# inverted-ai/torchdriveenv

Measured on AMD Instinct MI355X. Metric: env-steps/sec, higher is better.
Workload: dtype f32

## Files before the change

### torchdriveenv_amd/csrc/tde_device.h

```cpp
#pragma once
#include <hip/hip_runtime.h>
#include <stdint.h>

#include "../../include/tde_abi.h"

#define TDE_DEV __device__ __forceinline__

typedef uint32_t u32x4_t __attribute__((ext_vector_type(4)));

namespace tde {

constexpr float kPi = 3.14159265358979323846f;
constexpr float kTwoPi = 6.28318530717958647692f;
constexpr float k2OverPi = 0.636619772367581343f;
constexpr float kPio2A = 1.5703125f;
constexpr float kPio2B = 4.837512969970703125e-4f;
constexpr float kPio2C = 7.54978995489188216e-8f;

TDE_DEV uint32_t mask_lo(unsigned long long m) { return (uint32_t)m; }
TDE_DEV uint32_t mask_hi(unsigned long long m) { return (uint32_t)(m >> 32); }
TDE_DEV bool upper_half(int i)
{
    int up = i & 32;
    asm("" : "+v"(up));
// ... 143 lines not shown

TDE_DEV float seg_d2_inv(float px, float py, float ax, float ay, float bx, float by, float inv)
{
    float abx = bx - ax, aby = by - ay;
    float apx = px - ax, apy = py - ay;
    float t = (apx * abx + apy * aby) * inv;
    t = clampf(t, 0.0f, 1.0f);
    float qx = apx - t * abx, qy = apy - t * aby;
    return qx * qx + qy * qy;
}

TDE_DEV float point_tri_d2_words(float px, float py, const float4 &t0, const float4 &t1, const float4 &t2)
{
    const float ax = t0.x, ay = t0.y, bx = t0.z, by = t0.w, cx = t1.x, cy = t1.y;
    float e0 = (bx - ax) * (py - ay) - (by - ay) * (px - ax);
    float e1 = (cx - bx) * (py - by) - (cy - by) * (px - bx);
    float e2 = (ax - cx) * (py - cy) - (ay - cy) * (px - cx);
    if ((e0 >= 0.0f && e1 >= 0.0f && e2 >= 0.0f) || (e0 <= 0.0f && e1 <= 0.0f && e2 <= 0.0f)) return 0.0f;
    float d = seg_d2_inv(px, py, ax, ay, bx, by, t1.z);
    d = fminf(d, seg_d2_inv(px, py, bx, by, cx, cy, t1.w));
    d = fminf(d, seg_d2_inv(px, py, cx, cy, ax, ay, t2.x));
    return d;
}

TDE_DEV float point_tri_d2_packed(float px, float py, const float4 *__restrict__ T)
{
    const float4 t0 = T[0], t1 = T[1];
    const float ax = t0.x, ay = t0.y, bx = t0.z, by = t0.w, cx = t1.x, cy = t1.y;
    float e0 = (bx - ax) * (py - ay) - (by - ay) * (px - ax);
    float e1 = (cx - bx) * (py - by) - (cy - by) * (px - bx);
    float e2 = (ax - cx) * (py - cy) - (ay - cy) * (px - cx);
    if ((e0 >= 0.0f && e1 >= 0.0f && e2 >= 0.0f) || (e0 <= 0.0f && e1 <= 0.0f && e2 <= 0.0f)) return 0.0f;
    const float inv_ca = T[2].x;
    float d = seg_d2_inv(px, py, ax, ay, bx, by, t1.z);
    d = fminf(d, seg_d2_inv(px, py, bx, by, cx, cy, t1.w));
    d = fminf(d, seg_d2_inv(px, py, cx, cy, ax, ay, inv_ca));
    return d;
}

TDE_DEV uint32_t cell_lookup(const tde_world &w, const tde_map &m, float px, float py)
{
    const float fx = __builtin_amdgcn_fmed3f((px - m.ox) * m.inv_cell, 0.0f, (float)(m.nx - 1));
    const float fy = __builtin_amdgcn_fmed3f((py - m.oy) * m.inv_cell, 0.0f, (float)(m.ny - 1));
    return w.cell_word[(uint32_t)m.cell_base + (((uint32_t)(int)fy << m.row_shift) + (uint32_t)(int)fx)];
}

template <typename T> TDE_DEV T sel4(int i, T a0, T a1, T a2, T a3)
{
    const bool b0 = (i & 1) != 0, b1 = (i & 2) != 0;
    const T lo = b0 ? a1 : a0, hi = b0 ? a3 : a2;
    return b1 ? hi : lo;
}
#define TDE_SEL4(i, a0, a1, a2, a3) sel4((i), (a0), (a1), (a2), (a3))

struct Corners {
    float px0, py0, px1, py1, px2, py2, px3, py3;
    uint32_t w0, w1, w2, w3;
};

TDE_DEV uint32_t cell_class_lookup(const tde_world &w, const tde_map &m, float px, float py)
{
    const float fx = __builtin_amdgcn_fmed3f((px - m.ox) * m.inv_cell, 0.0f, (float)(m.nx - 1));
    const float fy = __builtin_amdgcn_fmed3f((py - m.oy) * m.inv_cell, 0.0f, (float)(m.ny - 1));
    const uint32_t ix = (uint32_t)(int)fx, iy = (uint32_t)(int)fy;
    const uint32_t tile = (uint32_t)m.cls2_base + ((iy >> 4) << (m.row_shift - 5)) + (ix >> 5);
    const uint32_t word = w.cell_cls2[(tile << 5) | (((iy & 15u) << 1) | ((ix >> 4) & 1u))];
    return ((word >> ((ix & 15u) << 1)) & 3u) | (((uint32_t)m.cell_base + ((iy << m.row_shift) + ix)) << 2);
}

#ifndef TDE_STEP_CLS2
#define TDE_STEP_CLS2 1
#endif
#ifndef TDE_ROLLOUT_CLS2
#define TDE_ROLLOUT_CLS2 0
#endif

template <bool CLS2 = false>
TDE_DEV void offroad_issue(const tde_world &w, const tde_map &m, bool live, float x, float y, float c, float s, float hl,
                           float hw, Corners &k)
{
    const float lx = hl * c, ly = hl * s, wx = hw * s, wy = hw * c;
    k.px0 = (x + lx) - wx; k.py0 = (y + ly) + wy;
    k.px1 = (x + lx) + wx; k.py1 = (y + ly) - wy;
    k.px2 = (x - lx) + wx; k.py2 = (y - ly) - wy;
    k.px3 = (x - lx) - wx; k.py3 = (y - ly) + wy;
    k.w0 = k.w1 = k.w2 = k.w3 = TDE_CELL_FULL;
    if (live) {
        if constexpr (CLS2) {
            k.w0 = cell_class_lookup(w, m, k.px0, k.py0);
            k.w1 = cell_class_lookup(w, m, k.px1, k.py1);
            k.w2 = cell_class_lookup(w, m, k.px2, k.py2);
            k.w3 = cell_class_lookup(w, m, k.px3, k.py3);
        } else {
            k.w0 = cell_lookup(w, m, k.px0, k.py0);
            k.w1 = cell_lookup(w, m, k.px1, k.py1);
            k.w2 = cell_lookup(w, m, k.px2, k.py2);
            k.w3 = cell_lookup(w, m, k.px3, k.py3);
        }
    }
}

template <bool PAIR = false, bool CLS2 = false>
TDE_DEV bool offroad_resolve(const tde_world &w, const Corners &k, float thr2, int rec_base)
{
    const uint32_t w0 = k.w0, w1 = k.w1, w2 = k.w2, w3 = k.w3;
    static_assert(TDE_CELL_EMPTY == 0u && TDE_CELL_MIXED == 1u && TDE_CELL_FULL == 2u, "cell classes");
    bool off = min(min(w0 & 3u, w1 & 3u), min(w2 & 3u, w3 & 3u)) == 0u;
    uint32_t pending = off ? 0u : ((w0 & 1u) | ((w1 & 1u) << 1) | ((w2 & 1u) << 2) | ((w3 & 1u) << 3));
    bool work = false;
    uint32_t cur = 0, end = 0;
    float qx = 0.0f, qy = 0.0f;
    const float4 *recs = reinterpret_cast<const float4 *>(w.cell_tri);
    for (;;) {
        if (!work && pending) {
            const int ci = __ffs((int)pending) - 1;
            pending &= pending - 1u;
            uint32_t wd = TDE_SEL4(ci, w0, w1, w2, w3);
            if constexpr (CLS2) wd = w.cell_word[wd >> 2];
            cur = (wd >> 10) + (uint32_t)rec_base;
            end = cur + ((wd >> 2) & 255u);
            qx = TDE_SEL4(ci, k.px0, k.px1, k.px2, k.px3);
            qy = TDE_SEL4(ci, k.py0, k.py1, k.py2, k.py3);
            work = true;
        }
        if (!__ballot(work)) break;
        if (work) {
            if constexpr (PAIR) {
                const float4 *r0 = recs + 3 * (size_t)cur, *r1 = recs + 3 * (size_t)(cur + 1 < end ? cur + 1 : cur);
                const float4 a0 = r0[0], a1 = r0[1], a2 = r0[2], b0 = r1[0], b1 = r1[1], b2 = r1[2];
                bool on = point_tri_d2_words(qx, qy, a0, a1, a2) <= thr2;
                if (!on && cur + 1 < end) on = point_tri_d2_words(qx, qy, b0, b1, b2) <= thr2;
                cur += 2;
                if (on) work = false;
                else if (cur >= end) { off = true; work = false; pending = 0u; }
            } else {
                const float d2 = point_tri_d2_packed(qx, qy, recs + 3 * (size_t)cur);
                if (d2 <= thr2) work = false;
                else if (++cur == end) { off = true; work = false; pending = 0u; }
            }
        }
    }
    return off;
}

template <bool PAIR = false, bool CLS2 = false>
TDE_DEV bool box_offroad(const tde_world &w, const tde_map &m, bool live, float x, float y, float c, float s, float hl,
                         float hw, float thr2)
{
    Corners k;
    offroad_issue<CLS2>(w, m, live, x, y, c, s, hl, hw, k);
    return offroad_resolve<PAIR, CLS2>(w, k, thr2, m.rec_base);
}

TDE_DEV uint4 philox(uint64_t seed, uint32_t c0, uint32_t c1, uint32_t c2, uint32_t c3)
{
    uint32_t k0 = (uint32_t)seed, k1 = (uint32_t)(seed >> 32);
#pragma unroll
    for (int r = 0; r < 10; ++r) {
        uint32_t h0 = __umulhi(0xD2511F53u, c0), l0 = 0xD2511F53u * c0;
        uint32_t h1 = __umulhi(0xCD9E8D57u, c2), l1 = 0xCD9E8D57u * c2;
        uint32_t n0 = h1 ^ c1 ^ k0, n2 = h0 ^ c3 ^ k1;
        c0 = n0; c1 = l1; c2 = n2; c3 = l0;
        k0 += 0x9E3779B9u; k1 += 0xBB67AE85u;
    }
    return make_uint4(c0, c1, c2, c3);
}

TDE_DEV double u01(uint32_t r) { return (double)(r >> 8) * (1.0 / 16777216.0); }

struct Sliver { double lo, hi; };
__host__ TDE_DEV Sliver sliver_of(double r) { const double r2 = r * r; return Sliver{r2 * (1.0 - 1e-12), r2 * (1.0 + 1e-12)}; }
TDE_DEV bool sqrt_gt(double s, double r, const Sliver &v)
{
    if (s > v.hi) return true;
    if (s < v.lo) return false;
    return sqrt(s) > r;
}
TDE_DEV bool sqrt_ge(double s, double r, const Sliver &v)
{
    if (s > v.hi) return true;
    if (s < v.lo) return false;
    return sqrt(s) >= r;
}

TDE_DEV double cos_kernel_f64(double x, double y)
{
    const double z = x * x;
    const double r = z * __builtin_fma(z, __builtin_fma(z, __builtin_fma(z, __builtin_fma(z, __builtin_fma(z,
                         -1.13596475577881948265e-11, 2.08757232129817482790e-09), -2.75573143513906633035e-07),
                         2.48015872894767294178e-05), -1.38888888888741095749e-03), 4.16666666666666019037e-02);
    const double hz = 0.5 * z, w = 1.0 - hz;
    return w + (((1.0 - w) - hz) + (z * r - x * y));
}
TDE_DEV double sin_kernel_f64(double x, double y)
{
    const double z = x * x, v = z * x;
    const double r = __builtin_fma(z, __builtin_fma(z, __builtin_fma(z, __builtin_fma(z, 1.58969099521155010221e-10,
                         -2.50507602534068634195e-08), 2.75573137070700676789e-06), -1.98412698298579493134e-04),
                         8.33333333332248946124e-03);
    return x - ((z * (0.5 * y - v * r) - y) - v * -1.66666666666666324348e-01);
}
TDE_DEV double cos_heading_f64(double x)
{
    if (__builtin_fabs(x) < 0.78539816339744830962) return cos_kernel_f64(x, 0.0);
    const double fn = __builtin_rint(x * 6.36619772367581382433e-01);
    const int n = (int)fn;
    const double r = x - fn * 1.57079632673412561417e+00, w = fn * 6.07710050650619224932e-11;
    const double y0 = r - w, y1 = (r - y0) - w;
    const double v = (n & 1) ? sin_kernel_f64(y0, y1) : cos_kernel_f64(y0, y1);
    return (((n + 1) & 2) != 0) ? -v : v;
}

__host__ TDE_DEV void cut2f_bounds(double r, float &lo, float &hi)
{
    const double r2 = r * r;
    lo = 0.0f; hi = __builtin_inff();
    if (r2 > 1e-30 && r2 < 1e30) { lo = (float)(r2 * (1.0 - 1e-6)); hi = (float)(r2 * (1.0 + 1e-6)); }
}

struct Cold {
    double waypoint_bonus, heading_penalty, distance_bonus, distance_cutoff, reach_radius;
    Sliver cut_sliver, reach_sliver;
    float cut2f_lo, cut2f_hi;
    uint64_t seed;
    const tde_spawn *spawn;
    const tde_scenario *scn;
    const double *wp_xy;
    const tde_map *maps;
    const float *route_xy;
    const float *start_psi;
    uint32_t env_base;
    int n_scn, NW, RW, max_steps, terminated_at_infraction, NH;
};

__host__ TDE_DEV void fill_cold(Cold &c, const tde_config &cfg, const tde_world &w)
{
    c.waypoint_bonus = cfg.waypoint_bonus; c.heading_penalty = cfg.heading_penalty;
    c.distance_bonus = cfg.distance_bonus; c.distance_cutoff = cfg.distance_cutoff;
    c.reach_radius = cfg.reach_radius; c.seed = cfg.seed;
    c.cut_sliver = sliver_of(cfg.distance_cutoff); c.reach_sliver = sliver_of(cfg.reach_radius);
    cut2f_bounds(cfg.distance_cutoff, c.cut2f_lo, c.cut2f_hi);
    c.spawn = w.spawn; c.scn = w.scn; c.wp_xy = w.wp_xy; c.maps = w.maps; c.route_xy = w.route_xy;
    c.start_psi = w.start_psi; c.NH = w.NH;
    c.env_base = cfg.env_base; c.n_scn = w.n_scn; c.NW = w.NW; c.RW = w.RW;
    c.max_steps = cfg.max_steps; c.terminated_at_infraction = cfg.terminated_at_infraction;
}

struct RewardBounds { Sliver cut, reach; float cut2f_lo, cut2f_hi; };
TDE_DEV RewardBounds reward_bounds(const Cold &c) { return RewardBounds{c.cut_sliver, c.reach_sliver, c.cut2f_lo, c.cut2f_hi}; }
TDE_DEV RewardBounds reward_bounds(const tde_config &c)
{
    RewardBounds b{sliver_of(c.distance_cutoff), sliver_of(c.reach_radius), 0.0f, 0.0f};
    cut2f_bounds(c.distance_cutoff, b.cut2f_lo, b.cut2f_hi);
    return b;
}

struct RewardOut {
    float reward;
    uint8_t terminated, truncated;
    double psi_smooth, speed_smooth, psi_r, dist_r;
};

template <typename CFG>
TDE_DEV double reward_dist_term(const CFG &cfg, const RewardBounds &rb, float lx, float ly, float x, float y)
{
    const float fdx = x - lx, fdy = y - ly;
    const float s32 = fdx * fdx + fdy * fdy;
    bool moved = s32 > rb.cut2f_hi;
    if (!moved && !(s32 < rb.cut2f_lo)) {
        const double ddx = (double)x - (double)lx, ddy = (double)y - (double)ly;
        moved = sqrt_gt(ddx * ddx + ddy * ddy, cfg.distance_cutoff, rb.cut);
    }
    return moved ? cfg.distance_bonus : 0.0;
}
template <typename CFG> TDE_DEV double reward_psi_term(const CFG &cfg, float lpsi, float psi)
{
    const float dpsi = psi - lpsi;
    return (1.0 - cos_heading_f64((double)dpsi)) * (-cfg.heading_penalty);
}
template <typename CFG>
TDE_DEV void reward_motion_terms(const CFG &cfg, const RewardBounds &rb, float lx, float ly, float lpsi, float x, float y,
                                 float psi, double &dist_r, double &psi_r)
{
    dist_r = reward_dist_term(cfg, rb, lx, ly, x, y);
    psi_r = reward_psi_term(cfg, lpsi, psi);
}
template <typename CFG>
TDE_DEV bool reward_reach(const CFG &cfg, const RewardBounds &rb, float x, float y, double wtx, double wty)
{
    const double tx = (double)x - wtx, ty = (double)y - wty;
    return !sqrt_ge(tx * tx + ty * ty, cfg.reach_radius, rb.reach);
}
template <typename CFG> TDE_DEV float reward_sum(const CFG &cfg, bool reach, double dist_r, double psi_r)
{
    return (float)(((reach ? cfg.waypoint_bonus : 0.0) + dist_r) + psi_r);
}

template <typename CFG>
TDE_DEV RewardOut reward_core(const CFG &cfg, int n_wp, double wtx, double wty, float lx, float ly, float lpsi,
                              float lv, float x, float y, float psi, float v, bool off, bool col, bool tl, int k,
                              int &target_idx, int &reached, bool want_info = true)
{
    RewardOut o;
    const RewardBounds rb = reward_bounds(cfg);
    reward_motion_terms(cfg, rb, lx, ly, lpsi, x, y, psi, o.dist_r, o.psi_r);
    const int ti = target_idx;
// ... 16 lines not shown
```

### torchdriveenv_amd/csrc/tde_kernels.h

```cpp
#ifndef TDE_KERNELS_H
#define TDE_KERNELS_H
#include <hip/hip_runtime.h>
#include <stdint.h>
#include <stdio.h>
#include <stdlib.h>
#include <string.h>
#include <atomic>
#include <type_traits>

#include "../../include/tde_hip.h"
#include "tde_device.h"
#include "tde_magnitudes.h"
#include "tde_raster.h"

#if (defined(TDE_EXP_NO_COLL_MAG) || defined(TDE_EXP_NO_OFF_MAG) || defined(TDE_EXP_EXTRA_LOAD) || defined(TDE_EXP_NO_D_RESPAWN) || \
     defined(TDE_EXP_NO_C_RESPAWN) || (defined(TDE_EXP_MAG_FRAME) && TDE_EXP_MAG_FRAME != 0)) && !defined(TDE_EXPERIMENT_BUILD)
#error "TDE_EXP_* switches build a library that computes WRONG results (timing experiments): add -DTDE_EXPERIMENT_BUILD to say you mean it"
#endif

namespace tde {

constexpr int kBlock = 256;
constexpr int kWave = 64;

// ... 1738 lines not shown
                if (F & TDE_F_REWARD) {
                    const float4 pa = sh.a[q][0], pc = sh.c[q][0];
                    int n_target = er.target_idx, n_reached = er.reached;
                    rw = reward_core(cold, cx.n_wp, cx.wtx, cx.wty, pa.x, pa.y, pc.x, pc.y, x, y, rc.x, rc.y, false, false, false, k,
                                     n_target, n_reached, st.info != nullptr);
                    const bool advanced = n_target != er.target_idx;
                    er.target_idx = n_target; er.reached = n_reached;
                    if (st.info) {
                        double *inf = st.info + 4 * (int64_t)e;
                        inf[0] = rw.psi_smooth; inf[1] = rw.speed_smooth; inf[2] = rw.psi_r; inf[3] = rw.dist_r;
                    }
                    if (st.info_reached) st.info_reached[e] = er.reached;
                    if (advanced) load_ego_target(cold, er, cx);
                    o.terminated = (uint8_t)(cold.terminated_at_infraction && (off || hit || tl));
                    o.truncated = (uint8_t)(k >= cold.max_steps);
                    done = (o.terminated | o.truncated) ? 1 : 0;
                }
                sh.done = ((F & TDE_F_REWARD) && (F & TDE_F_AUTORESET)) ? done : 0;
                if (ro.reward) ro.reward[(int64_t)i * LB + e] = rw.reward;
                if (ro.done)
                    ro.done[(int64_t)i * LB + e] =
                        (uint8_t)(o.terminated | (o.truncated << 1) | (o.offroad << 2) | (o.collided << 3) | (o.tl << 4));
            }
        }
        lds_barrier();
        const bool respawned = sh.done != 0;
        if (respawned) reset_lane<A>(cfg, cold, e, a, ag, er);
        st.collided[g] = respawned ? 0 : o.collided;
        st.offroad[g] = respawned ? 0 : o.offroad;
        if (a == 0) {
            st.scn[e] = er.scn; st.episode[e] = er.episode;
            st.steps[e] = er.steps;
            st.target_idx[e] = er.target_idx;
            st.reached[e] = er.reached;
            st.reward[e] = rw.reward;
            st.terminated[e] = o.terminated;
            st.truncated[e] = o.truncated;
            if (st.tl_violation) st.tl_violation[e] = o.tl;
        }
    } else if (NW == 8 && role == 2) {
        __builtin_amdgcn_s_setprio(3);
        if (lane == 0) sh.help_seq[wv & 1] = 0;
        lds_barrier();
        for (int i = 0; i < ro.K; ++i) {
            const int q = (i & 1) ^ 1;
            if (F & TDE_F_NPC) {
                const float4 ra = sh.a[q][a], rb = sh.b[q][a];
                const float gf = sh.ctl[a];
                Agent me{};
                me.x = ra.x; me.y = ra.y; me.len = 2.0f * rb.z;
                const unsigned long long own = one_bit64(63 - (a & 63));
                sh.gap_part[a] = npc_gap<64>(cfg, &sh.a[q][64], &sh.b[q][64], a - 64, a < 64 ? 0ull : own, me, rb.x, rb.y, gf >= 0.0f, gf);
                asm volatile("s_waitcnt lgkmcnt(0)" ::: "memory");
                if (lane == 0) *reinterpret_cast<volatile int *>(&sh.help_seq[wv & 1]) = i + 1;
            }
            lds_barrier();
            if (sh.done && first_acts) lds_barrier();
            lds_barrier();
        }
        lds_barrier();
    } else if (NW == 8 && role == 3) {
        __builtin_amdgcn_s_setprio(1);
        Agent ag{};
        EnvRegs er{st.scn[e], st.steps[e], st.target_idx[e], st.reached[e], st.episode[e]};
        RedCache redc; redc.invalidate();
        tde_map m{};
        if (F & (TDE_F_OFFROAD | TDE_F_TRAFFIC_LIGHTS)) m = cold.maps[reinterpret_cast<const int4 *>(cold.scn)[er.scn].x];
        const float thr2 = thr2_of(cfg);
        if (lane == 0) sh.off_seq[wv & 1] = 0;
        lds_barrier();
        for (int i = 0; i < ro.K; ++i) {
            const int p = i & 1;
            lds_barrier();
            if (sh.done) {
                reset_lane<A>(cfg, cold, e, a, ag, er);
                if (F & (TDE_F_OFFROAD | TDE_F_TRAFFIC_LIGHTS)) m = cold.maps[reinterpret_cast<const int4 *>(cold.scn)[er.scn].x];
                redc.invalidate();
                if (first_acts) lds_barrier();
            }
            lds_barrier();
            er.steps += 1;
            const float4 ra = sh.a[p][a], rb = sh.b[p][a], rc = sh.c[p][a];
            const bool live = rc.z != 0.0f;
            bool off = false;
            if (F & TDE_F_OFFROAD) {
                Corners corners;
                offroad_issue<false>(w, m, live, ra.x, ra.y, rb.x, rb.y, rb.z, rb.w, corners);
                off = offroad_resolve<false, false>(w, corners, thr2, m.rec_base);
            }
            sh.offw[a] = off ? 1 : 0;
            if (LIGHTS && (F & TDE_F_TRAFFIC_LIGHTS) && a == 0)
                sh.tlw = tl_violation_of(WideLines{sh, w.stoplines + m.stop_base}, m.n_stop, red_mask_cached(w, m, er.steps, redc), ra.x, ra.y, rb.x, rb.y, rb.z, rb.w) ? 1 : 0;
            asm volatile("s_waitcnt lgkmcnt(0)" ::: "memory");
            if (lane == 0) *reinterpret_cast<volatile int *>(&sh.off_seq[wv & 1]) = i + 1;
        }
        lds_barrier();
    }
}
#undef TDE_WIDE_PROLOGUE

#ifdef TDE_DEBUG
#ifndef TDE_DUMMY_D
#define TDE_DUMMY_D 0
#endif
#ifndef TDE_DUMMY_C
#define TDE_DUMMY_C 0
#endif
#ifndef TDE_DUMMY_O
#define TDE_DUMMY_O 0
#endif
#ifndef TDE_DUMMY_ILP
#define TDE_DUMMY_ILP 1
#endif
template <int N> TDE_DEV void dummy_valu(float seed)
{
    if constexpr (N > 0) {
        float v[TDE_DUMMY_ILP];
#pragma unroll
        for (int u = 0; u < TDE_DUMMY_ILP; ++u) v[u] = seed + (float)u;
#pragma unroll
        for (int n = 0; n < N / TDE_DUMMY_ILP; ++n) {
#pragma unroll
            for (int u = 0; u < TDE_DUMMY_ILP; ++u) asm volatile("v_fma_f32 %0, %0, %0, %0" : "+v"(v[u]));
        }
#pragma unroll
        for (int u = 0; u < TDE_DUMMY_ILP; ++u) asm volatile("" :: "v"(v[u]));
    }
}
#define TDE_PROBE(N, seed) dummy_valu<N>(seed)
#else
#define TDE_PROBE(N, seed) ((void)0)
#endif
#ifndef TDE_STEP_PRIO_SWITCH
#define TDE_STEP_PRIO_SWITCH 1
#endif
#ifndef TDE_STEP_PRIO_D2
#define TDE_STEP_PRIO_D2 0
#define TDE_STEP_PRIO_C2 3
#define TDE_STEP_PRIO_O2 2
#endif
#ifndef TDE_SPRIO_C
#define TDE_SPRIO_C 0
#define TDE_SPRIO_O 1
#endif
#ifndef TDE_PRIO_D
#define TDE_PRIO_D 2
#define TDE_PRIO_C 0
#define TDE_PRIO_O 1
#endif
#ifndef TDE_ROLLOUT_CONST_ARGS
#define TDE_ROLLOUT_CONST_ARGS 0
#endif
struct RolloutArgs { tde_config cfg; tde_world w; tde_state st; tde_rollout ro; uint32_t act_hash; };
#if TDE_ROLLOUT_CONST_ARGS
__constant__ RolloutArgs g_rollout_args;
#endif
template <int A, bool LIGHTS, bool BIG>
__global__ __launch_bounds__(3 * kWave) __attribute__((amdgpu_waves_per_eu(6, 6))) void env_rollout_trio_kernel(
#if TDE_ROLLOUT_CONST_ARGS
    int unused_)
{
    const tde_config &cfg = g_rollout_args.cfg; const tde_world &w = g_rollout_args.w; const tde_state &st = g_rollout_args.st;
    const tde_rollout &ro = g_rollout_args.ro;
    const uint32_t act_hash = g_rollout_args.act_hash;
#else
    tde_config cfg, tde_world w, tde_state st, tde_rollout ro, uint32_t act_hash)
{
#endif
    __shared__ DuoShared sh;
    __shared__ Cold cold;
    const int lane = threadIdx.x & (kWave - 1);
    const int role = __builtin_amdgcn_readfirstlane((int)(threadIdx.x >> 6));
    if (threadIdx.x == 0) {
        fill_cold(cold, cfg, w); sh.done = 0ull; sh.hit_mask = 0ull; sh.off_mask = 0ull; sh.tl_mask = 0ull;
        sh.max_steps_w = cfg.max_steps; sh.term_at_infraction_w = cfg.terminated_at_infraction;
        sh.red_seq = -1;
    }
    const uint32_t F = cfg.flags;
    const bool lights = LIGHTS && (F & TDE_F_TRAFFIC_LIGHTS);
    constexpr bool kGapCache = TDE_FIRST_GAP != 0 && LIGHTS;
    const bool first_acts = (F & TDE_F_NPC_FIRST_STEP) != 0;
    const int64_t g = (int64_t)blockIdx.x * kWave + lane;
    const int e = (int)(g / A), a = (int)(g % A);
    const int B = st.B;
    const int LB = ro.ldb;
    const bool valid = e < B;
    const int64_t gs = valid ? g : 0;
    const int es = valid ? e : 0;
    const int base = lane - a;
    __syncthreads();
#define TDE_ROLE_PROLOGUE                                                                                 \
    Agent ag;                                                                                             \
    load_agent(st, gs, ag);                                                                               \
    if (!valid) ag.present = false;                                                                       \
    EnvRegs er{st.scn[es], st.steps[es], st.target_idx[es], st.reached[es], st.episode[es]};              \
    Ctx cx;                                                                                               \
    load_ctx<A>(cfg, cold, a, ag, er, cx);

    uint4 m0, m1;
    auto done_of = [&](int k, unsigned long long &term_m, unsigned long long &trunc_m) {
        const unsigned long long ego = __ballot(a == 0 && valid);
        m0 = *reinterpret_cast<const uint4 *>(&sh.hit_mask);
        m1 = *reinterpret_cast<const uint4 *>(&sh.tl_mask);
        const unsigned long long infr = (((unsigned long long)(m0.y | m0.w | m1.y)) << 32) | (m0.x | m0.z | m1.x);
        term_m = ((F & TDE_F_REWARD) && m1.w) ? (infr & ego) : 0ull;
        trunc_m = (F & TDE_F_REWARD) ? __ballot(a == 0 && valid && k >= (int)m1.z) : 0ull;
        return ((F & TDE_F_REWARD) && (F & TDE_F_AUTORESET)) ? (term_m | trunc_m) : 0ull;
    };
    if (role == 0) {
        TDE_ROLE_PROLOGUE
        __builtin_amdgcn_s_setprio(TDE_PRIO_D);
        float c0, s0;
        sincos_f32(ag.psi, s0, c0);
        write_rows(sh, 1, lane, valid && ag.present, ag, c0, s0, cfg.npc_lane_half);
        lds_barrier();
        for (int i = 0; i < ro.K; ++i) {
            const int p = i & 1, q = p ^ 1;
            const float2 act = sh.act[p][base];
            float nx, ny, npsi, nv, nc, ns;
            float na = 0.0f, nb = 0.0f;
            int nwp, k;
            bool switched, live;
            bool again = false;
            for (int pass = 0;; ++pass) {
                k = er.steps + 1;
                live = valid && ag.present;
                const bool npc = (F & TDE_F_NPC) && a > 0 && live;
                const bool replayed = (F & TDE_F_REPLAY) && a > 0 && live && k < cx.replay_len;
                float4 rep = make_float4(0.0f, 0.0f, 0.0f, 0.0f);
                if (replayed) rep = reinterpret_cast<const float4 *>(w.replay_states)[(int64_t)ag.replay * w.RT + k];
                const bool has_target = npc && ag.route >= 0 && ag.route_wp < cx.route_n;
                float acc = 0.0f, beta = 0.0f;
                if (a == 0) { acc = act.x; beta = act.y; }
                if (F & TDE_F_NPC) {
                    if (pass == 0 || again) {
                        const float gap = npc_gap<A>(cfg, &sh.a[q][base], &sh.b[q][base], a, bit_of_row<A>(a), ag, c0, s0, has_target, cx.g_far);
                        float red_gap = 1e30f;
                        if (lights) {
                            if (pass == 0) {
                                while (*reinterpret_cast<volatile int *>(&sh.red_seq) != i) __builtin_amdgcn_s_sleep(1);
                                red_gap = *reinterpret_cast<volatile float *>(&sh.red_gap[p][lane]);
                            } else if (has_target) {
                                const tde_map m = cold.maps[reinterpret_cast<const int4 *>(cold.scn)[er.scn].x];
                                const uint32_t red = red_mask(w, m, k);
                                if (red) red_gap = red_line_gap_of<GlobalLines, 1>(cfg, GlobalLines{w.stoplines + m.stop_base}, m.n_stop, red, ag, c0, s0);
                            }
                        }
                        npc_act_of_gap(cfg, ag, c0, s0, has_target, cx.tgx, cx.tgy, gap, has_target ? red_gap : 1e30f, na, nb);
                    }
                    if (npc && (k > 1 || first_acts)) { acc = na; beta = nb; }
                }
                nx = ag.x; ny = ag.y; npsi = ag.psi; nv = ag.v;
                if (live) {
                    bicycle(nx, ny, npsi, nv, ag.inv_lr, acc, beta, cfg.dt);
                    if (replayed) { nx = rep.x; ny = rep.y; npsi = rep.z; nv = rep.w; }
                }
                switched = false;
                nwp = ag.route_wp;
                if (has_target) {
                    const float dx = cx.tgx - nx, dy = cx.tgy - ny;
                    if (dx * dx + dy * dy < cfg.npc_reach * cfg.npc_reach) { nwp += 1; switched = true; }
                }
                sincos_f32(npsi, ns, nc);
                TDE_PROBE(TDE_DUMMY_D, nx);
                if (pass) break;
                lds_barrier();
                unsigned long long term_m, trunc_m;
                const unsigned long long dn = i > 0 ? done_of(er.steps, term_m, trunc_m) : 0ull;
                if (lane == 0) sh.done = dn;
                if (!dn) break;
                const bool fresh = mask_bit(dn, base) && valid;
                uint2 fg_ent = make_uint2(0u, 0u);
                if (fresh) {
                    reset_lane<A>(cfg, cold, e, a, ag, er);
                    if (kGapCache && first_acts && (F & TDE_F_NPC) && a > 0 && w.first_gap)
                        fg_ent = *reinterpret_cast<const uint2 *>(w.first_gap + ((int64_t)er.scn * A + a));
                    load_ctx<A>(cfg, cold, a, ag, er, cx);
                    sincos_f32(ag.psi, s0, c0);
                    write_rows(sh, q, lane, ag.present, ag, c0, s0, cfg.npc_lane_half);
                }
                if (first_acts && (F & TDE_F_NPC)) {
                    again = true;
                    if constexpr (kGapCache) {
                        const bool f_npc = fresh && a > 0 && ag.present;
                        const bool f_target = f_npc && ag.route >= 0 && ag.route_wp < cx.route_n;
                        again = !npc_first_step<A>(cfg, fg_ent, first_gap_key(act_hash), &sh.a[q][base], &sh.b[q][base], a, ag, c0, s0, f_npc, f_target,
                                                   cx.tgx, cx.tgy, na, nb);
                    }
                }
            }
            ag.x = nx; ag.y = ny; ag.psi = npsi; ag.v = nv; ag.route_wp = nwp;
            c0 = nc; s0 = ns;
            er.steps = k;
            write_rows(sh, p, lane, live, ag, c0, s0, cfg.npc_lane_half);
            lds_barrier();
            if (switched) load_route_target(cold, ag, cx);
        }
        lds_barrier();
        {
            unsigned long long term_m, trunc_m;
            const unsigned long long dn = done_of(er.steps, term_m, trunc_m);
            if (lane == 0) sh.done = dn;
            lds_barrier();
            if (mask_bit(dn, base) && valid) reset_lane<A>(cfg, cold, e, a, ag, er);
        }
        if (!valid) return;
        store_agent_dynamic(st, g, ag);
        store_agent_static(st, g, ag);
    } else if (role == 1) {
        __builtin_amdgcn_s_setprio(TDE_PRIO_C);
        TDE_ROLE_PROLOGUE
        RedCache redc; redc.invalidate();
        bool hit = false;
        uint8_t last_term = 0, last_trunc = 0;
        int npend = 0, ipend0 = 0;
        const bool batch = (F & TDE_F_REWARD) != 0;
        if (batch) load_ego_ctx(cold, er, cx);
        auto flush = [&](bool final) {
            const int n = npend;
            if (n == 0) return;
            const bool act = valid && a < n;
            const float4 r0 = sh.ring_pre[lane], r1 = sh.ring_post[lane];
            const RewardBounds rbn = reward_bounds(cold);
            double dist_r = 0.0, psi_r = 0.0;
            if (act) reward_motion_terms(cold, rbn, r0.x, r0.y, r0.z, r1.x, r1.y, r1.z, dist_r, psi_r);
            int from = 0;
            for (;;) {
                bool reach = false;
                if (act && a >= from && er.target_idx < cx.n_wp) reach = reward_reach(cold, rbn, r1.x, r1.y, cx.wtx, cx.wty);
                const unsigned long long rm = __ballot(reach);
                const uint32_t envbits = mask_field(rm, base) & (A >= 32 ? 0xffffffffu : ((1u << (A & 31)) - 1u));
                const int s1 = envbits ? __ffs((int)envbits) - 1 : A;
                if (act && a >= from && a <= s1) {
                    const float rwd = reward_sum(cold, a == s1, dist_r, psi_r);
                    if (ro.reward) ro.reward[(int64_t)(ipend0 + a) * LB + e] = rwd;
                    if (final && a == n - 1) {
                        st.reward[e] = rwd;
                        if (st.info) {
                            double *inf = st.info + 4 * (int64_t)e;
                            inf[0] = (double)fabsf((r0.z - r1.z) / 0.1f); inf[1] = (double)fabsf((r0.w - r1.w) / 0.1f);
                            inf[2] = psi_r; inf[3] = dist_r;
                        }
                    }
                }
                bool more = false;
                if (s1 < A) {
                    er.target_idx += 1; er.reached += 1;
                    load_ego_target(cold, er, cx);
                    from = s1 + 1;
                    more = valid && from < n;
                } else {
                    from = n;
                }
                if (!__ballot(more)) break;
            }
            if (final && a == 0 && valid && st.info_reached) st.info_reached[e] = er.reached;
            ipend0 += n; npend = 0;
        };
        auto settle = [&](int i) {
            unsigned long long term_m, trunc_m;
            const unsigned long long dn = done_of(er.steps, term_m, trunc_m);
            if (a == 0 && valid) {
                last_term = (uint8_t)mask_bit(term_m, lane); last_trunc = (uint8_t)mask_bit(trunc_m, lane);
                if (ro.done) {
                    const bool up = lane >= 32;
                    const uint32_t sft = (uint32_t)lane & 31u;
                    const uint32_t hb = ((up ? m0.y : m0.x) >> sft) & 1u, ob = ((up ? m0.w : m0.z) >> sft) & 1u,
                                   tb = ((up ? m1.y : m1.x) >> sft) & 1u;
                    ro.done[(int64_t)i * LB + e] = (uint8_t)(last_term | (last_trunc << 1) | (ob << 2) | (hb << 3) | (tb << 4));
                }
            }
            return dn;
        };
        auto publish_red_gaps = [&](int step, int buf, int kk) {
            __builtin_amdgcn_s_setprio(3);
            const float4 ra = sh.a[buf][lane], rb = sh.b[buf][lane];
            float rg = 1e30f;
            const uint32_t red = red_mask_cached(w, cx.m, kk, redc);
            if (red) {
                Agent me{};
                me.x = ra.x; me.y = ra.y; me.len = 2.0f * rb.z;
                if (cx.m.n_stop <= kStopCache)
                    rg = red_line_gap_of<CacheOnlyLines<A>, TDE_JUDGE_GAP_LINES>(cfg, CacheOnlyLines<A>{sh, lane / A}, cx.m.n_stop, red, me, rb.x, rb.y);
                else
                    rg = red_line_gap_of<CachedLines<A>, TDE_JUDGE_GAP_LINES>(cfg, CachedLines<A>{sh, w.stoplines + cx.m.stop_base, lane / A}, cx.m.n_stop, red, me, rb.x, rb.y);
            }
            sh.red_gap[step & 1][lane] = rg;
            if (a == 0) sh.lights2[step & 1][lane / A] = make_int4((int)red, 0, cx.m.stop_base, cx.m.n_stop);
            asm volatile("s_waitcnt lgkmcnt(0)" ::: "memory");
            if (lane == 0) *reinterpret_cast<volatile int *>(&sh.red_seq) = step;
            __builtin_amdgcn_s_setprio(TDE_PRIO_C);
        };
        if (lights) fill_stop_cache<A>(sh, w, cx.m, lane, a);
        lds_barrier();
        if (lights) publish_red_gaps(0, 1, er.steps + 1);
        for (int i = 0; i < ro.K; ++i) {
            const int p = i & 1, q = p ^ 1;
            lds_barrier();
            if (i > 0) {
                const unsigned long long dn = settle(i - 1);
                if (dn && batch) flush(false);
                if (dn && mask_bit(dn, base) && valid) {
                    reset_lane<A>(cfg, cold, e, a, ag, er);
                    load_ctx<A>(cfg, cold, a, ag, er, cx);
                    if (batch) load_ego_ctx(cold, er, cx);
                    redc.invalidate();
                    if (lights) {
                        fill_stop_cache<A>(sh, w, cx.m, lane, a);
                        if (a == 0) sh.lights2[p][lane / A] = make_int4((int)red_mask_cached(w, cx.m, 1, redc), 0, cx.m.stop_base, cx.m.n_stop);
                    }
                }
            }
            lds_barrier();
            er.steps += 1;
            const int k = er.steps;
            if (lights && i + 1 < ro.K) publish_red_gaps(i + 1, p, k + 1);
            const float4 ra = sh.a[p][lane], rb = sh.b[p][lane], rc = sh.c[p][lane];
            if constexpr (A == 16 && TDE_COLLIDE_DPP)
                hit = collide_rows_dpp16(&sh.a[p][base], &sh.b[p][base], a, rc.z != 0.0f, ra.x, ra.y, rb.x, rb.y, rb.z, rb.w, ra.z);
            else
                hit = collide_rows<A>(&sh.a[p][base], &sh.b[p][base], a, rc.z != 0.0f, ra.x, ra.y, rb.x, rb.y, rb.z, rb.w, ra.z);
            const unsigned long long m = __ballot(hit);
            if (lane == 0) sh.hit_mask = m;
            TDE_PROBE(TDE_DUMMY_C, ra.x);
            if (batch) {
                if (a == 0 && valid) {
                    const float4 pa = sh.a[q][lane], pc = sh.c[q][lane];
                    sh.ring_pre[lane + npend] = make_float4(pa.x, pa.y, pc.x, pc.y);
                    sh.ring_post[lane + npend] = make_float4(ra.x, ra.y, rc.x, rc.y);
                }
                npend += 1;
                if (npend == A && i + 1 < ro.K) flush(false);
            } else if (a == 0 && valid && ro.reward) {
                ro.reward[(int64_t)i * LB + e] = 0.0f;
            }
        }
        lds_barrier();
        settle(ro.K - 1);
        if (batch) flush(true);
        lds_barrier();
        const bool respawned = mask_bit(sh.done, base) != 0;
        if (respawned && valid) reset_lane<A>(cfg, cold, e, a, ag, er);
        if (!valid) return;
        st.collided[g] = respawned ? 0 : (hit ? 1 : 0);
        if (a == 0) {
            st.scn[e] = er.scn; st.episode[e] = er.episode;
            st.steps[e] = er.steps;
            st.target_idx[e] = er.target_idx;
            st.reached[e] = er.reached;
            if (!batch) st.reward[e] = 0.0f;
            st.terminated[e] = last_term;
            st.truncated[e] = last_trunc;
        }
    } else {
        __builtin_amdgcn_s_setprio(TDE_PRIO_O);
        TDE_ROLE_PROLOGUE
        const float thr2 = thr2_of(cfg);
        bool off = false, tl = false;
        const float2 *acts = reinterpret_cast<const float2 *>(ro.actions);
        const bool ego = a == 0 && valid;
        if (ego) {
            sh.act[0][lane] = acts[e];
            sh.act[1][lane] = acts[(int64_t)(ro.K > 1 ? 1 : 0) * LB + e];
        }
        lds_barrier();
        for (int i = 0; i < ro.K; ++i) {
            const int p = i & 1;
            float2 act2 = make_float2(0.0f, 0.0f);
            if (ego) act2 = acts[(int64_t)(i + 2 < ro.K ? i + 2 : ro.K - 1) * LB + e];
            lds_barrier();
            lds_barrier();
            if (i > 0) {
                const unsigned long long dn = sh.done;
                if (dn && mask_bit(dn, base) && valid) {
                    reset_lane<A>(cfg, cold, e, a, ag, er);
                    load_ctx<A>(cfg, cold, a, ag, er, cx);
                }
            }
            er.steps += 1;
            const int k = er.steps;
            const float4 ra = sh.a[p][lane], rb = sh.b[p][lane], rc = sh.c[p][lane];
            const bool live = rc.z != 0.0f;
            off = false;
            if (F & TDE_F_OFFROAD) off = box_offroad<false, BIG || TDE_ROLLOUT_CLS2>(w, cx.m, live, ra.x, ra.y, rb.x, rb.y, rb.z, rb.w, thr2);
            tl = false;
            if (lights && a == 0 && valid) {
                const int4 lw = sh.lights2[p][lane / A];
                if (lw.w <= kStopCache) tl = tl_violation_of(CacheOnlyLines<A>{sh, lane / A}, lw.w, (uint32_t)lw.x, ra.x, ra.y, rb.x, rb.y, rb.z, rb.w);
                else tl = tl_violation_of(CachedLines<A>{sh, w.stoplines + lw.z, lane / A}, lw.w, (uint32_t)lw.x, ra.x, ra.y, rb.x, rb.y, rb.z, rb.w);
            }
            TDE_PROBE(TDE_DUMMY_O, ra.x);
            const unsigned long long om = __ballot(off), tm = __ballot(tl);
            if (lane == 0) { sh.off_mask = om; sh.tl_mask = tm; }
            if (ego) sh.act[p][lane] = act2;
        }
        lds_barrier();
        lds_barrier();
        if (!valid) return;
        st.offroad[g] = mask_bit(sh.done, base) ? 0 : (off ? 1 : 0);
        if (a == 0 && st.tl_violation) st.tl_violation[e] = tl ? 1 : 0;
    }
}
#undef TDE_ROLE_PROLOGUE

TDE_DEV void load_next_target(const Cold &w, const Agent &ag, int route_n, float &x2, float &y2)
{
    x2 = y2 = 0.0f;
    if (ag.route >= 0 && ag.route_wp + 1 < route_n) {
        const float2 tg = reinterpret_cast<const float2 *>(w.route_xy)[(int64_t)ag.route * w.RW + ag.route_wp + 1];
        x2 = tg.x; y2 = tg.y;
    }
}

constexpr uint32_t kSlotKeyFlags = TDE_F_NPC | TDE_F_REPLAY;
constexpr int kSlotTg2Later = 1 << 29;

TDE_DEV int slot_key(const Agent &ag, uint32_t F)
{
    return (ag.route_wp & 0xFFFF) | (int)((F & kSlotKeyFlags) << 16) | TDE_CACHE_VALID;
}

template <int A>
TDE_DEV void load_ctx_cached(const tde_config &cfg, const Cold &cold, const tde_state &st, int64_t g, int a, bool valid,
                             const int4 &s0, const int4 &s1, Agent &ag, const EnvRegs &er, Ctx &cx,
                             bool want_map, bool &rebuilt)
{
    const uint32_t F = cfg.flags;
    const bool hit = !valid || (s0.x == er.scn && (s0.y & ~kSlotTg2Later) == slot_key(ag, F));
    rebuilt = !hit;
    cx.wtx = cx.wty = 0.0; cx.n_wp = 0;
    cx.tgx2 = cx.tgy2 = 0.0f;
    if (__ballot(!hit)) {
        if (!hit) {
            load_ctx<A>(cfg, cold, a, ag, er, cx);
            load_next_target(cold, ag, cx.route_n, cx.tgx2, cx.tgy2);
        }
    }
    if (hit) {
        cx.tgx = __int_as_float(s0.z); cx.tgy = __int_as_float(s0.w);
        constexpr uint32_t idm = (1u << TDE_CACHE_ID_BITS) - 1u;
        ag.route = (int)((uint32_t)s1.x & idm) - 1; cx.route_n = (int)((uint32_t)s1.x >> TDE_CACHE_ID_BITS);
        ag.replay = (int)((uint32_t)s1.y & idm) - 1; cx.replay_len = (int)((uint32_t)s1.y >> TDE_CACHE_ID_BITS);
        cx.tgx2 = __int_as_float(s1.z); cx.tgy2 = __int_as_float(s1.w);
        cx.g_far = (ag.vdes * ag.vdes / cfg.npc_max_accel) * 1.01f + cfg.npc_gap_s0 + 0.1f;
        if (want_map && (F & (TDE_F_OFFROAD | TDE_F_TRAFFIC_LIGHTS))) {
            const int4 e0 = reinterpret_cast<const int4 *>(st.env_cache + (g / A))[0];
            const int map = ((e0.z & TDE_CACHE_VALID) && e0.x == er.scn) ? e0.w : reinterpret_cast<const int4 *>(cold.scn)[er.scn].x;
            cx.m = cold.maps[map];
        }
    }
}

TDE_DEV void store_slot_cache(const tde_state &st, int64_t g, const Agent &ag, const EnvRegs &er, const Ctx &cx, uint32_t F,
                              bool tg2_later = false)
{
    static_assert(sizeof(tde_slot_cache) == 32, "two 16-byte words per slot");
    int4 *sc4 = reinterpret_cast<int4 *>(st.slot_cache + g);
    sc4[0] = make_int4(er.scn, slot_key(ag, F) | (tg2_later ? kSlotTg2Later : 0), __float_as_int(cx.tgx), __float_as_int(cx.tgy));
    sc4[1] = make_int4((int)((uint32_t)(ag.route + 1) | ((uint32_t)cx.route_n << TDE_CACHE_ID_BITS)),
                       (int)((uint32_t)(ag.replay + 1) | ((uint32_t)cx.replay_len << TDE_CACHE_ID_BITS)),
                       __float_as_int(cx.tgx2), __float_as_int(cx.tgy2));
}

TDE_DEV int act_key_steps(uint32_t cfg_hash, int steps) { return (int)(cfg_hash ^ ((uint32_t)steps * 0x9E3779B1u)); }


#ifndef TDE_WIDE_PRIO_D2
#define TDE_WIDE_PRIO_D2 3
#endif
#ifndef TDE_WIDE_PRIO_J2
#define TDE_WIDE_PRIO_J2 1
#endif
#ifndef TDE_WIDE4_SWEEP_BLOCK
#define TDE_WIDE4_SWEEP_BLOCK 4
#endif
#ifndef TDE_WIDE_STEP_WAVES8
#define TDE_WIDE_STEP_WAVES8 1
#endif
struct WideStepShared : WideShared {
    int early[2];
    float poly[32];
};

template <bool LIGHTS, bool OBS, bool MAG, int NW = 4>
__global__ __launch_bounds__(NW * kWave) __attribute__((amdgpu_waves_per_eu(4, 4))) void env_step_wide_kernel(const StepArgs *__restrict__ args,
                                                                                                           const float *__restrict__ action)
{
    const tde_config &cfg = args->cfg;
    const tde_world &w = args->w;
    const tde_state &st = args->st;
    const uint32_t act_hash = args->act_hash;
    constexpr int A = 128;
    __shared__ WideStepShared sh;
#if TDE_WIDE_COLD_IN_BLOCK
    const Cold &cold = args->cold;
#define TDE_WIDE_COLD_BARRIER() ((void)0)
#else
    __shared__ Cold cold;
#define TDE_WIDE_COLD_BARRIER() lds_barrier()
#endif
    const int lane = threadIdx.x & (kWave - 1);
    const int wv = wide_role_wave();
    const int role = wv >> 1;
    const int a = ((wv & 1) << 6) | lane;
#if !TDE_WIDE_COLD_IN_BLOCK
    if (wv == (NW == 8 ? 4 : 2) && lane == 0) fill_cold(cold, cfg, w);
#endif
    const uint32_t F = cfg.flags;
    const bool first_acts = (F & TDE_F_NPC_FIRST_STEP) != 0;
    const bool lights = LIGHTS && (F & TDE_F_TRAFFIC_LIGHTS);
    const int e = (int)blockIdx.x;
    const int64_t g = (int64_t)e * A + a;
    if (role == 0) {
        __builtin_amdgcn_s_setprio(2);
        Agent ag;
        load_agent(st, g, ag);
        EnvRegs er{st.scn[e], st.steps[e], st.target_idx[e], st.reached[e], st.episode[e]};
        const float2 act = reinterpret_cast<const float2 *>(action)[e];
        float2 ac = make_float2(0.0f, 0.0f);
        int2 akey = make_int2(-1, 0);
        float2 *ap = st.act_cache ? reinterpret_cast<float2 *>(st.act_cache) + (int64_t)e * (A + 1) : nullptr;
        if (ap) { ac = ap[a]; akey = reinterpret_cast<const int2 *>(ap)[A]; }
        int4 sc0 = make_int4(0, 0, 0, 0), sc1 = sc0;
        if (st.slot_cache) { sc0 = reinterpret_cast<const int4 *>(st.slot_cache + g)[0]; sc1 = reinterpret_cast<const int4 *>(st.slot_cache + g)[1]; }
        TDE_WIDE_COLD_BARRIER();
        Ctx cx;
        bool rebuilt;
        load_ctx_cached<A>(cfg, cold, st, g, a, true, sc0, sc1, ag, er, cx, false, rebuilt);
        if (!rebuilt && lights) cx.m = cold.maps[reinterpret_cast<const int4 *>(cold.scn)[er.scn].x];
        const bool need_tg2 = !rebuilt && (sc0.y & kSlotTg2Later) != 0;
        const bool live = ag.present;
        const int k = er.steps + 1;
        const bool npc = (F & TDE_F_NPC) && a > 0 && live;
        const bool replayed = (F & TDE_F_REPLAY) && a > 0 && live && k < cx.replay_len;
        float4 rep = make_float4(0.0f, 0.0f, 0.0f, 0.0f);
        if (replayed) rep = reinterpret_cast<const float4 *>(w.replay_states)[(int64_t)ag.replay * w.RT + k];
        bool has_target = npc && ag.route >= 0 && ag.route_wp < cx.route_n;
        float acc = 0.0f, beta = 0.0f;
        if (a == 0) { acc = act.x; beta = act.y; }
        float c0, s0;
        auto controller = [&](int buf, int kk, float &na, float &nb) {
            const uint32_t red = lights ? red_mask(w, cx.m, kk) : 0u;
            const float red_gap = (lights && red && has_target) ? red_line_gap_of(cfg, WideLines{sh, w.stoplines + cx.m.stop_base}, cx.m.n_stop, red, ag, c0, s0) : 1e30f;
            npc_action_wide<A, (NW == 4 && !LIGHTS && !MAG) ? TDE_WIDE4_SWEEP_BLOCK : kSweepBlock>(cfg, &sh.a[buf][0], &sh.b[buf][0], a, ag, c0, s0, has_target, cx.tgx, cx.tgy,
                                                                                          cx.g_far, red_gap, na, nb);
// ... 1034 lines not shown
```

Baseline: 2.753 billion.

## Compute only ego collision and offroad on intermediate rollout steps

On every rollout step except the last, the collision and offroad roles now evaluate only what the ego agent needs. Collision runs one pairwise test per lane against the ego, and offroad splits the ego's four box corners across lanes 0..3. The results are ORed into the ego lane's bit of each env via a shift-fold of the ballot mask. This removes the all-pairs collision rows and the per-agent offroad box checks on steps where only ego termination and reward matter. The cost is that the masks no longer carry per-NPC flags on intermediate steps, so any consumer that reads non-ego bits there would see different values.

New measurement: 3.161 billion (median of 6 runs). 1.15x the previous value.

```diff
diff --git a/torchdriveenv_amd/csrc/tde_device.h b/torchdriveenv_amd/csrc/tde_device.h
--- a/torchdriveenv_amd/csrc/tde_device.h
+++ b/torchdriveenv_amd/csrc/tde_device.h
@@ -319,6 +319,27 @@
     return offroad_resolve<PAIR, CLS2>(w, k, thr2, m.rec_base);
 }
 
+template <bool CLS2 = false>
+TDE_DEV bool corner_offroad(const tde_world &w, const tde_map &m, int i, float x, float y, float c, float s, float hl, float hw,
+                            float thr2)
+{
+    const float lx = hl * c, ly = hl * s, wx = hw * s, wy = hw * c;
+    const bool front = i < 2, right = i == 1 || i == 2;
+    const float px = (x + (front ? lx : -lx)) + (right ? wx : -wx);
+    const float py = (y + (front ? ly : -ly)) + (right ? -wy : wy);
+    uint32_t wd = CLS2 ? cell_class_lookup(w, m, px, py) : cell_lookup(w, m, px, py);
+    const uint32_t cls = wd & 3u;
+    if (cls != TDE_CELL_MIXED) return cls == TDE_CELL_EMPTY;
+    if constexpr (CLS2) wd = w.cell_word[wd >> 2];
+    uint32_t cur = (wd >> 10) + (uint32_t)m.rec_base;
+    const uint32_t end = cur + ((wd >> 2) & 255u);
+    const float4 *recs = reinterpret_cast<const float4 *>(w.cell_tri);
+    do {
+        if (point_tri_d2_packed(px, py, recs + 3 * (size_t)cur) <= thr2) return false;
+    } while (++cur != end);
+    return true;
+}
+
 TDE_DEV uint4 philox(uint64_t seed, uint32_t c0, uint32_t c1, uint32_t c2, uint32_t c3)
 {
     uint32_t k0 = (uint32_t)seed, k1 = (uint32_t)(seed >> 32);
diff --git a/torchdriveenv_amd/csrc/tde_kernels.h b/torchdriveenv_amd/csrc/tde_kernels.h
--- a/torchdriveenv_amd/csrc/tde_kernels.h
+++ b/torchdriveenv_amd/csrc/tde_kernels.h
@@ -1914,6 +1914,12 @@
 #define TDE_ROLLOUT_CONST_ARGS 0
 #endif
 struct RolloutArgs { tde_config cfg; tde_world w; tde_state st; tde_rollout ro; uint32_t act_hash; };
+template <int A> TDE_DEV unsigned long long fold_env_to_ego(unsigned long long m)
+{
+#pragma unroll
+    for (int s = 1; s < A; s <<= 1) m |= m >> s;
+    return m;
+}
 #if TDE_ROLLOUT_CONST_ARGS
 __constant__ RolloutArgs g_rollout_args;
 #endif
@@ -1939,6 +1945,7 @@
         sh.red_seq = -1;
     }
     const uint32_t F = cfg.flags;
+    constexpr bool kEgoJudgeC = A <= 16, kEgoJudgeO = A <= 16 && !LIGHTS;
     const bool lights = LIGHTS && (F & TDE_F_TRAFFIC_LIGHTS);
     constexpr bool kGapCache = TDE_FIRST_GAP != 0 && LIGHTS;
     const bool first_acts = (F & TDE_F_NPC_FIRST_STEP) != 0;
@@ -2178,11 +2185,25 @@
             const int k = er.steps;
             if (lights && i + 1 < ro.K) publish_red_gaps(i + 1, p, k + 1);
             const float4 ra = sh.a[p][lane], rb = sh.b[p][lane], rc = sh.c[p][lane];
-            if constexpr (A == 16 && TDE_COLLIDE_DPP)
-                hit = collide_rows_dpp16(&sh.a[p][base], &sh.b[p][base], a, rc.z != 0.0f, ra.x, ra.y, rb.x, rb.y, rb.z, rb.w, ra.z);
-            else
-                hit = collide_rows<A>(&sh.a[p][base], &sh.b[p][base], a, rc.z != 0.0f, ra.x, ra.y, rb.x, rb.y, rb.z, rb.w, ra.z);
-            const unsigned long long m = __ballot(hit);
+            unsigned long long m;
+            if (kEgoJudgeC && i + 1 < ro.K) {
+                const float4 ea = sh.a[p][base];
+                const float dx = ra.x - ea.x, dy = ra.y - ea.y, rr = ea.z + ra.z;
+                const float dy2 = dy * dy;
+                const float v = __builtin_fmaf(-rr, rr, __builtin_fmaf(dx, dx, dy2));
+                bool pair = false;
+                if (a > 0 && (__float_as_uint(v) >> 31) && sh.c[p][base].z != 0.0f) {
+                    const float4 eb = sh.b[p][base];
+                    pair = obb_overlap(ea.x, ea.y, eb.x, eb.y, eb.z, eb.w, ra.x, ra.y, rb.x, rb.y, rb.z, rb.w);
+                }
+                m = fold_env_to_ego<A>(__ballot(pair));
+            } else {
+                if constexpr (A == 16 && TDE_COLLIDE_DPP)
+                    hit = collide_rows_dpp16(&sh.a[p][base], &sh.b[p][base], a, rc.z != 0.0f, ra.x, ra.y, rb.x, rb.y, rb.z, rb.w, ra.z);
+                else
+                    hit = collide_rows<A>(&sh.a[p][base], &sh.b[p][base], a, rc.z != 0.0f, ra.x, ra.y, rb.x, rb.y, rb.z, rb.w, ra.z);
+                m = __ballot(hit);
+            }
             if (lane == 0) sh.hit_mask = m;
             TDE_PROBE(TDE_DUMMY_C, ra.x);
             if (batch) {
@@ -2244,7 +2265,20 @@
             const float4 ra = sh.a[p][lane], rb = sh.b[p][lane], rc = sh.c[p][lane];
             const bool live = rc.z != 0.0f;
             off = false;
-            if (F & TDE_F_OFFROAD) off = box_offroad<false, BIG || TDE_ROLLOUT_CLS2>(w, cx.m, live, ra.x, ra.y, rb.x, rb.y, rb.z, rb.w, thr2);
+            unsigned long long om = 0ull;
+            if (F & TDE_F_OFFROAD) {
+                if (kEgoJudgeO && i + 1 < ro.K) {
+                    bool corner = false;
+                    if (a < 4 && sh.c[p][base].z != 0.0f) {
+                        const float4 ea = sh.a[p][base], eb = sh.b[p][base];
+                        corner = corner_offroad<BIG || TDE_ROLLOUT_CLS2>(w, cx.m, a, ea.x, ea.y, eb.x, eb.y, eb.z, eb.w, thr2);
+                    }
+                    om = fold_env_to_ego<A>(__ballot(corner));
+                } else {
+                    off = box_offroad<false, BIG || TDE_ROLLOUT_CLS2>(w, cx.m, live, ra.x, ra.y, rb.x, rb.y, rb.z, rb.w, thr2);
+                    om = __ballot(off);
+                }
+            }
             tl = false;
             if (lights && a == 0 && valid) {
                 const int4 lw = sh.lights2[p][lane / A];
@@ -2252,7 +2286,7 @@
                 else tl = tl_violation_of(CachedLines<A>{sh, w.stoplines + lw.z, lane / A}, lw.w, (uint32_t)lw.x, ra.x, ra.y, rb.x, rb.y, rb.z, rb.w);
             }
             TDE_PROBE(TDE_DUMMY_O, ra.x);
-            const unsigned long long om = __ballot(off), tm = __ballot(tl);
+            const unsigned long long tm = __ballot(tl);
             if (lane == 0) { sh.off_mask = om; sh.tl_mask = tm; }
             if (ego) sh.act[p][lane] = act2;
         }
```
